# InternLM/lmdeploy

Measured on AMD Instinct MI355X. Metric: decode tokens/sec, Llama-3-8B W4A16 int8-KV batch 64 (1024-in/1k-out synthetic), higher is better.
Workload: dtype f16; 1 GPU; Llama-3-8B shapes, W4A16 AWQ g128 random weights, quant_policy=8 KV, batch 64, 1024-token random prompts, greedy decode, TP=1; batch=64, prompt_len=1024, parallelism=tp1, collectives=none, rccl_ranks=0, decode_splits=1, hipgraph=True, rmsnorm_fold=0, gemm_dispatch=measured at start-up (tm_engine_tune_gemm), prefill_rows=8192

## Files before the change

### lmdeploy_amd/csrc/c_api.hip

```cpp
#include "../../include/tm_mi355x.h"
#include "scheduler.h"
#define TM_TRY_RC(expr)          \
    do {                        \
        const int _rc = (expr); \
        if (_rc) {              \
            return _rc;         \
        }                       \
    } while (0)
#include "tm_common.h"
#include "tm_kernels.h"
#include <string.h>
#include <cmath>
#include <vector>

namespace tmk {

static thread_local std::string g_last_error;

void set_last_error(const std::string& msg)
{
    g_last_error = msg;
}
const char* get_last_error()
{
// ... 285 lines not shown

int tm_linear_dequant_f16(const tm_linear* w, void* out_nk, tm_stream_t st)
{
    TM_REQUIRE(w && out_nk, "null pointer");
    return launch_dequant_p32_f16((half_t*)out_nk, w->w, (hipStream_t)st);
}


int tm_linear_forward(const tm_linear* w, const void* x, int ldx, void* y, int ldy, int M, int gated_silu, int nt,
                      int splits, int waves, void* workspace, tm_stream_t st)
{
    TM_REQUIRE(w && x && y, "null pointer");
    GemmConfig cfg = gemm_pick_config(w->w, M);
    if (nt > 0) {
        cfg.nt = nt;
    }
    if (splits > 0) {
        cfg.splits = splits;
    }
    if (nt > 0 || (waves > 0 && !(waves & 0x200))) {
        cfg.d32_shape = -1;
        if (splits <= 0) {
            cfg.splits = gemm_pick_config_general(w->w, M).splits;
        }
    }
    if (waves > 0 && (waves & 0x200) && (waves & 0xff) == kShapeF16 && !w->w.image16) {
        TM_TRY_RC(linear_weight_build_f16_image(const_cast<tm_linear*>(w)->w, (hipStream_t)st));
    }
    if (waves > 0 && (waves & 0x200)) {
        TM_REQUIRE(dec32_supported(w->w, M), "decode kernel: u4 weights, N % 32 == 0");
        cfg.d32_shape = waves & 0xff;
        TM_REQUIRE((cfg.d32_shape >= 6 && cfg.d32_shape <= 9) || (cfg.d32_shape <= 5 && (cfg.d32_shape >= 4) == (M > 64))
                       || (cfg.d32_shape == kShapeWide2 && M <= 64)
                       || (cfg.d32_shape == kShapeLC && M <= 64) || ((cfg.d32_shape == kShapePre256 || cfg.d32_shape == kShapeF16) && M > 64)
                       || (dec32_is_merge_shape(cfg.d32_shape) && M <= 64),
                   "P32 kernel shape 0..3 / 11 (M <= 64), 4 / 5 / 12 (M > 64), 6..9 (32-row blocks, any M) or 16 + (0..3 | 6..9) "
                   "(M <= 64: split-K merged inside the launch)");
        waves = 0;
    }
    if (dec32_is_merge_shape(cfg.d32_shape) && workspace && cfg.splits > 1) {
        cfg.tickets = (unsigned*)((char*)workspace + gemm_workspace_bytes(M, w->w.N, 16));
        TM_HIP_CHECK(hipMemsetAsync(cfg.tickets, 0, 8192, (hipStream_t)st));
    }
    if (waves > 0) {
        TM_REQUIRE((waves & 0xff) == 4 || (waves & 0xff) == 8 || (waves & 0xff) == 16,
                   "waves in {4, 8, 16} (+0x100: two k-phases)");
        cfg.waves   = waves & 0xff;
        cfg.kphases = (waves & 0x100) ? 2 : 1;
    }
    TM_REQUIRE(cfg.splits <= 16, "splits <= 16");
    if (!workspace) {
        cfg.splits = 1;
    }
    return launch_linear(w->w, (const half_t*)x, ldx, (half_t*)y, ldy, M, gated_silu != 0, cfg, (float*)workspace, false,
                         nullptr, (hipStream_t)st);
}

int tm_linear_residual_norm(const tm_linear* w, const void* x, int ldx, void* y, void* resid, const void* norm_w, float eps, int M,
                            int shape, int splits, void* workspace, tm_stream_t st)
{
    TM_REQUIRE(w && x && y && resid && norm_w && workspace, "null pointer");
    const int N = w->w.N;
    GemmConfig cfg = gemm_pick_config(w->w, M);
    if (shape >= 0) {
        TM_REQUIRE(dec32_supported(w->w, M) && (shape <= 3 || (shape >= 6 && shape <= 10) || shape == kShapeLC)
                       && (M <= 64 || (M <= kFoldMaxRows && shape >= 6 && shape <= 9)),
                   "decode tile 0..3 / 6..10 / 11 at M <= 64; the 32-row-block tiles 6..9 up to 128 rows");
        cfg.d32_shape = shape;
    }
// ... 677 lines not shown
```

### lmdeploy_amd/csrc/gemm_decode.hip

```cpp
#include "tm_common.h"
#include "tm_kernels.h"
#include "p32_layout.h"
#include "gemm_decode_common.h"
#include <stdlib.h>
#include <algorithm>
#include <type_traits>
#include <map>
#include <mutex>
#include <string>
#include <tuple>
#include <stdio.h>

namespace tmk {

__global__ void repack_p32_kernel(uint32_t* __restrict__ out, const int32_t* __restrict__ qw, const half_t* __restrict__ scales,
                                  const half_t* __restrict__ zeros, int K, int N)
{
    const size_t idx   = (size_t)blockIdx.x * blockDim.x + threadIdx.x;
    const int    ncg   = N / 32;
    const size_t total = (size_t)(K / 128) * ncg * (kP32Unit / 4);
    if (idx >= total) {
        return;
    }
    const size_t unit = idx / (kP32Unit / 4);
// ... 1074 lines not shown
            }
            return launch_dec32_one<MH, 4, 4, 4, 2, kD32Mode>(p, grid, st);
        }
        case 1:
            return launch_dec32_one<MH, 8, 2, 4, 4, kD32Mode>(p, grid, st);
        case 2:
            return launch_dec32_one<MH, 4, 2, 4, 4, kD32Mode>(p, grid, st);
        case 3:
            if constexpr (l2pf_compiled) {
                if (l2pf == 1) return launch_dec32_one<MH, 2, 4, 4, 2, kD32Mode | 0x4000>(p, grid, st);
                if (l2pf == 2) return launch_dec32_one<MH, 2, 4, 4, 2, kD32Mode | 0x8000>(p, grid, st);
            }
            return launch_dec32_one<MH, 2, 4, 4, 2, kD32Mode>(p, grid, st);
        case kShapeWide2:
            return launch_dec32_one<MH, 8, 2, 2, 2, kD32Mode>(p, grid, st);
        default: break;
    }
    set_last_error("gemm_dec32: unknown shape");
    return 1;
}

static int dec32_base_shape(int shape)
{
    static const int base[4] = {3, 0, 2, 1};
    if (dec32_is_merge_shape(shape)) {
        shape -= kShapeMerge;
    }
    return shape >= 6 && shape <= 9 ? base[shape - 6] : shape;
}

static void dec32_shape_dims(int shape, int* cg, int* s)
{
    static const int cgs[6] = {4, 8, 4, 2, 8, 16};
    if (shape == kShapeLC) {
        *cg = 4;
        *s  = 4;
        return;
    }
    if (shape == kShapePre256 || shape == kShapeF16) {
        *cg = 8;
        *s  = 1;
        return;
    }
    shape = dec32_base_shape(shape);
    if (shape == kShapeWide2) {
        *cg = 8;
        *s  = 2;
        return;
    }
    *cg = cgs[shape < 0 || shape > 5 ? 0 : shape];
    *s  = shape == 5 ? 1 : (shape == 4 ? 2 : 4);
}

static bool dec32_on(bool big)
{
    static const int on     = env_int2("TM_GEMM_D32", 1);
    static const int on_big = env_int2("TM_GEMM_D32_PREFILL", 1);
    return on && (!big || on_big);
}

bool dec32_supported(const LinearWeight& w, int M)
{
    return dec32_on(M > 64) && w.type == 0 && w.packed32 != nullptr && M >= 1 && w.N % 32 == 0 && w.K % 128 == 0;
}

bool dec32_serves_every_m(int K, int N)
{
// ... 46 lines not shown
                kv.second.second, std::get<0>(kv.first));
    }
    gen_table_export_lines(f);
    fclose(f);
    return 0;
}

int dec32_table_import(const char* path)
{
    FILE* f = fopen(path, "r");
    if (!f) {
        set_last_error(std::string("cannot read ") + path);
        return 1;
    }
    int  K, N, M, shape, splits, n = 0, skipped = 0;
    char line[160];
    while (fgets(line, sizeof line, f)) {
        if (line[0] == 'G') {
            const bool ok = gen_table_import_line(line);
            n += ok ? 1 : 0;
            skipped += ok ? 0 : 1;
            continue;
        }
        if (line[0] == '#' || line[0] == '\n') {
            continue;
        }
        int       role = 0;
        const int got  = sscanf(line, "%d %d %d %d %d %d", &K, &N, &M, &shape, &splits, &role);
        if (got < 5 || role < 0 || role > 4) {
            ++skipped;
            continue;
        }
        const bool big = M > 64;
        const bool lc  = shape == kShapeLC && M <= 64;
        const bool p256 = (shape == kShapePre256 || (shape == kShapeF16 && splits == 1)) && M > 64;
        const bool mrg = dec32_is_merge_shape(shape) && M <= 64 && splits >= 2;
        const bool w2k = shape == kShapeWide2 && M <= 64;
        if (K > 0 && N > 0 && M > 0 && M == dec32_m_bucket(M) && shape >= 0 && (shape <= 9 || lc || p256 || mrg || w2k) && splits >= 1 && splits <= 16
            && (big ? shape >= 4 : (shape != 4 && shape != 5)) && !(shape == 5 && N < 512) && K % 128 == 0 && N % 32 == 0) {
            dec32_table_set(K, N, M, shape, splits, role);
            ++n;
        }
        else {
            ++skipped;
        }
    }
    fclose(f);
    if (skipped) {
        fprintf(stderr, "[tm] %s: %d dispatch line(s) not understood by this build were skipped (%d imported)\n", path, skipped, n);
    }
    return n > 0 ? 0 : 1;
}

int dec32_m_bucket(int M)
{
    if (M <= 256) {
        return M;
    }
    int b = 512;
    while (b < M && b < 8192) {
        b <<= 1;
    }
    return b;
}

int dec32_candidates(const LinearWeight& w, int M, int (*out)[2], int cap)
{
// ... 12 lines not shown
        }
        int       cgn, S;
        dec32_shape_dims(shape, &cgn, &S);
        const int tiles = (ncg + cgn - 1) / cgn * (rows32 ? (M + 31) / 32 : (shape == 4 || shape == 5) ? (M + 127) / 128 : 1);
        for (int s = 1; s <= 16; ++s) {
            int per = (KB + s - 1) / s;
            per     = (per + S - 1) / S * S;
            if ((KB + per - 1) / per != s) {
                continue;
            }
            if ((s > 1 && tiles * s > (rows32 ? 512 : 320)) || tiles * s < 32 || (M > 256 && s > 4)) {
                continue;
            }
            if (n < cap) {
                out[n][0] = shape;
                out[n][1] = s;
                ++n;
            }
        }
    }
    if (M <= 64) {
        const int base = n;
        for (int i = 0; i < base; ++i) {
            const int sh = out[i][0], sp = out[i][1];
            if (dec32_fold_shape(sh) && sh < kShapeMerge && sp >= 2 && sp <= 4 && n < cap) {
                out[n][0] = kShapeMerge + sh;
                out[n][1] = sp;
                ++n;
            }
        }
    }
    if (M <= 64) {
        const int tiles = (ncg + 3) / 4;
        for (int s = 1; s <= 16; ++s) {
            int per = (KB + s - 1) / s;
            per     = (per + 3) / 4 * 4;
            if ((KB + per - 1) / per != s || (s > 1 && tiles * s > 320) || tiles * s < 32) {
                continue;
            }
            if (n < cap) {
                out[n][0] = kShapeLC;
                out[n][1] = s;
                ++n;
            }
        }
    }
    if (M >= 1024 && M <= 8192 && w.N >= 256 && w.image16 != nullptr && n < cap) {
        out[n][0] = kShapeF16;
        out[n][1] = 1;
        ++n;
    }
    if (M >= 256 && M <= 8192 && w.N >= 256) {
        const int tiles = (ncg + 7) / 8 * ((M + 255) / 256);
        for (int s = 1; s <= 4; ++s) {
            const int per = (KB + s - 1) / s;
            if ((KB + per - 1) / per != s || (s > 1 && tiles * s > 512) || per < 8) {
                continue;
            }
            if (n < cap) {
                out[n][0] = kShapePre256;
                out[n][1] = s;
                ++n;
            }
        }
    }
    return n;
}

void dec32_pick(const LinearWeight& w, int M, int* shape_out, int* splits_out)
{
    dec32_pick_ex(w, M, shape_out, splits_out, true);
}

void dec32_pick_ex(const LinearWeight& w, int M, int* shape_out, int* splits_out, bool use_table)
{
    const int ncg = w.N / 32;
// ... 61 lines not shown
    }
    return M <= kFoldMaxRows && ((shape >= 6 && shape <= 9) || (shape == 4 && !producer));
}

bool dec32_fold_shape(int shape)
{
    if (dec32_is_merge_shape(shape)) {
        shape -= kShapeMerge;
    }
    return (shape >= 0 && shape <= 3) || (shape >= 6 && shape <= 9) || shape == kShapeWide2;
}

int launch_linear_dec32(const LinearWeight& w, const half_t* x, int ldx, half_t* y, int ldy, int M, bool gated_silu, int shape,
                        int splits, float* workspace, int* slabs_out, hipStream_t st, NormFold* nf)
{
    const bool produce = nf && nf->resid != nullptr;
    const bool consume = nf && nf->ss_in != nullptr;
    bool       merge   = false;
    if (dec32_is_merge_shape(shape)) {
        shape -= kShapeMerge;
        merge = !produce && splits > 1;
        TM_REQUIRE(!merge || (nf && nf->tickets && (M <= 64 || (M <= kFoldMaxRows && shape >= 6 && shape <= 9))),
                   "merged split-K: arrival counters (NormFold::tickets), M <= 64 (32-row-block tiles: <= 128)");
    }
    TM_REQUIRE(!nf || !(produce || consume)
                   || (M <= 64 ? dec32_fold_shape(shape) : (M <= kFoldMaxRows && ((shape >= 6 && shape <= 9) || (shape == 4 && !produce)))),
               "folded RMSNorm: decode tiles 0..3 / 6..10 at M <= 64; 32-row-block tiles 6..9 (and tile 4 as a consumer) up to 128 rows");
    TM_REQUIRE(!produce || (!gated_silu && nf->norm_w && nf->ss_out && ldy % 4 == 0), "folded RMSNorm, producer: residual, norm weight, sums");
    TM_REQUIRE(!consume || (nf->ss_tiles >= 1 && nf->inv_h > 0.f), "folded RMSNorm, consumer: tiles and 1 / H");
    TM_REQUIRE(w.packed32 != nullptr && w.N % 32 == 0, "decode GEMM: P32 layout missing");
    if (shape == kShapeF16 && (w.image16 == nullptr || M <= 64)) {
        shape = kShapePre256;
    }
    TM_REQUIRE(M >= 1 && shape >= 0 && (shape <= 9 || shape == kShapeWide2 || shape == kShapeLC || shape == kShapePre256 || shape == kShapeF16)
                   && (shape >= 6 || (M <= 64) == (shape < 4)) && (shape != kShapeLC || M <= 64) && (shape != kShapePre256 || M > 64)
                   && (shape != kShapeWide2 || M <= 64),
               "decode GEMM: shapes 0..3, 10 and 11 take M <= 64, shapes 4 / 5 / 12 take M > 64, shapes 6..9 any M");
    TM_REQUIRE(ldx % 8 == 0, "x rows must be 16-byte aligned");
    int cgn, S;
    dec32_shape_dims(shape, &cgn, &S);
    Dec32Params p{};
    p.x       = x;
    p.ldx     = ldx;
    p.wp      = shape == kShapeF16 ? (const void*)w.image16 : w.packed32;
    if (shape == kShapeF16) {
        splits = 1;
    }
    p.y       = y;
    p.ldy     = ldy;
    p.partial = workspace;
    p.M       = M;
    p.N       = w.N;
    p.K       = w.K;
    p.KB      = w.K / 128;
    p.ncg     = w.N / 32;
    int per   = (p.KB + splits - 1) / splits;
    per       = (per + S - 1) / S * S;
    per       = per > p.KB ? p.KB : per;
    splits    = (p.KB + per - 1) / per;
    TM_REQUIRE(splits == 1 || workspace != nullptr, "split-K needs a workspace");
    p.kb_per_split = per;
    merge          = merge && splits > 1;
    p.epilogue     = produce ? 3 : (splits > 1 && !merge) ? 2 : (gated_silu ? 1 : 0);
    if (merge) {
        p.merge   = 1;
        p.tickets = nf->tickets;
    }
    if (produce) {
        TM_REQUIRE(splits == 1 || nf->tickets != nullptr, "folded RMSNorm, producer with split-K: arrival counters");
        p.resid   = nf->resid;
        p.norm_w  = nf->norm_w;
        p.ss_out  = nf->ss_out;
        p.tickets = nf->tickets;
    }
    if (consume) {
        p.ss_in    = nf->ss_in;
        p.ss_tiles = nf->ss_tiles;
        p.ss_inv_h = nf->inv_h;
        p.ss_eps   = nf->eps;
    }
    static const int wt = env_int2("TM_D32_WT", 1);
    p.wt           = wt;
    dim3      grid((p.ncg + cgn - 1) / cgn, splits,
                   (shape == kShapePre256 || shape == kShapeF16) ? (M + 255) / 256 : (shape == kShapeLC || shape == kShapeWide2) ? 1 : shape >= 6 ? (M + 31) / 32 : shape >= 4 ? (M + 127) / 128 : 1);
    static const char* const role_tag[6] = {"gemm", "w_qkv", "wo", "w1w3", "w2", "lm_head"};
    p.dbg        = gemm_trace_for((size_t)grid.x * grid.y * grid.z, role_tag[w.role >= 0 && w.role <= 5 ? w.role : 0], grid.x, grid.y, grid.z);
    const int rc = shape == kShapeF16 ? launch_f16_256(p, grid, st) :
                   shape == kShapePre256 ? launch_pre256(p, grid, st) :
                   shape == kShapeLC ? launch_dec_lc(p, grid, st) :
                   shape == kShapeWide2 ? (M <= 32 ? launch_dec32_shape<1>(p, grid, shape, st) : launch_dec32_shape<2>(p, grid, shape, st)) :
                   shape >= 6 ? launch_dec32_shape<1>(p, grid, dec32_base_shape(shape), st) :
                   shape >= 4 ? launch_dec32_shape<4>(p, grid, shape, st) :
                   M <= 32    ? launch_dec32_shape<1>(p, grid, shape, st) :
                                launch_dec32_shape<2>(p, grid, shape, st);
    if (rc) {
        return rc;
    }
    if (produce) {
        nf->tiles_out = (int)grid.x;
        splits        = 1;
    }
    if (merge) {
        splits = 1;
    }
    if (slabs_out) {
        *slabs_out = splits;
    }
    return 0;
}

}
```

### lmdeploy_amd/csrc/gemm_decode_common.h

```cpp
#pragma once
#include "tm_common.h"
#include "tm_kernels.h"
#include "p32_layout.h"
#include <type_traits>

namespace tmk {

typedef float floatx16 __attribute__((ext_vector_type(16)));

struct Dec32Params {
    const half_t* x;
    int           ldx;
    const void*   wp;
    half_t*       y;
    int           ldy;
    float*        partial;
    int           M, N, K, KB, ncg;
    int           kb_per_split;
    int           epilogue;
    int           wt;
    uint64_t*     dbg;
    half_t*       resid;
    const half_t* norm_w;
    float*        ss_out;
// ... 19 lines not shown
{
    if (mode <= 1) {
        asm volatile("global_store_dwordx4 %0, %1, off sc1\n\ts_nop 1" ::"v"(dst), "v"(v) : "memory");
    }
    else if (mode == 2) {
        asm volatile("global_store_dwordx4 %0, %1, off sc0 sc1\n\ts_nop 1" ::"v"(dst), "v"(v) : "memory");
    }
    else if (mode == 3) {
        asm volatile("global_store_dwordx4 %0, %1, off nt\n\ts_nop 1" ::"v"(dst), "v"(v) : "memory");
    }
    else {
        asm volatile("global_store_dwordx4 %0, %1, off sc0 sc1 nt\n\ts_nop 1" ::"v"(dst), "v"(v) : "memory");
    }
}
__device__ __forceinline__ void store_wt(half4_t* dst, half4_t v)
{
    asm volatile("global_store_dwordx2 %0, %1, off sc1" ::"v"(dst), "v"(v) : "memory");
}
__device__ __forceinline__ void store_wt(half2_t* dst, half2_t v)
{
    asm volatile("global_store_dword %0, %1, off sc1" ::"v"(dst), "v"(v) : "memory");
}

template<int N, class F, int I = 0>
__device__ __forceinline__ void static_for(F&& f)
{
    if constexpr (I < N) {
        f(std::integral_constant<int, I>{});
        static_for<N, F, I + 1>(static_cast<F&&>(f));
    }
}

int launch_dec_lc(const Dec32Params& p, dim3 grid, hipStream_t st);
int launch_pre256(const Dec32Params& p, dim3 grid, hipStream_t st);
int launch_f16_256(const Dec32Params& p, dim3 grid, hipStream_t st);

}
```

### lmdeploy_amd/csrc/gemm_decode_lc.hip

```cpp
#include "gemm_decode_common.h"
#include <stdlib.h>

namespace tmk {

typedef float floatx2 __attribute__((ext_vector_type(2)));

__device__ __forceinline__ half8_t raw8_p32(uint32_t w)
{
    const uint32_t m = 0x000f000fu;
    return bit_cast<half8_t>(u32x4{w & m, (w >> 4) & m, (w >> 8) & m, (w >> 12) & m});
}

template<int MH, int PFS, int ABL = 0>
__global__ __launch_bounds__(768) void gemm_dec_lc_kernel(Dec32Params p)
{
    constexpr int NCW   = 2;
    constexpr int CGW   = 2;
    constexpr int WK    = 4;
    constexpr int NCONS = CGW * WK;
    constexpr int NLOAD = 4;
    constexpr int T     = (NCONS + NLOAD) * 64;
    constexpr int ROWS  = 32 * MH;
    constexpr int KBB   = ROWS * 256;
    constexpr int S     = WK;
    constexpr int STG   = S * KBB;
    constexpr int CGT   = CGW * NCW;
    constexpr int NPC   = S * ROWS / 4;
    constexpr int DR    = NPC / NLOAD;
    static_assert(NPC % NLOAD == 0, "DMA pieces per loader wave");
    static_assert(WK * ROWS * CGT * 128 <= 2 * STG, "reduction image must fit the stage buffers");

    extern __shared__ __attribute__((aligned(16))) char smem[];

    const int tid  = threadIdx.x;
    const int wgid = blockIdx.y * gridDim.x + blockIdx.x;
    if (p.dbg && tid == 0) {
        p.dbg[wgid * 8 + 0] = __builtin_amdgcn_s_memrealtime();
        p.dbg[wgid * 8 + 4] = ((uint64_t)__builtin_amdgcn_s_getreg(20 | (31 << 11)) << 32) | (uint32_t)__builtin_amdgcn_s_getreg(4 | (31 << 11));
    }
    const int lane = tid & 63;
    const int wave = __builtin_amdgcn_readfirstlane(tid >> 6);
    const int l31  = lane & 31;
    const int half = lane >> 5;

    const int kb0 = blockIdx.y * p.kb_per_split;
    const int nkb = min(p.kb_per_split, p.KB - kb0);
    const int nst = (nkb + S - 1) / S;
    const int Mloc = min(ROWS, p.M);

    const unsigned lds0 = __builtin_amdgcn_readfirstlane((unsigned)(size_t)smem);

    floatx16 acc[NCW][MH];
#pragma unroll
    for (int c = 0; c < NCW; ++c) {
// ... 193 lines not shown
                        }
                    }
                    if constexpr (!(ABL & (1 | 2))) {
#pragma unroll
                        for (int g = 0; g < 2 * MH; ++g) {
                            __builtin_amdgcn_sched_group_barrier(0x008, 1, 0);
                            __builtin_amdgcn_sched_group_barrier(0x002, MH == 2 ? 7 : 14, 0);
                        }
                    }
                    __builtin_amdgcn_sched_barrier(0);
                });
                if constexpr (!(ABL & 16)) {
                    LC_LOAD_W(u, (t + PFS) * S + wk);
                }
                __builtin_amdgcn_s_barrier();
            };
            int t0 = 0;
            for (; t0 + PFS <= nst; t0 += PFS) {
                static_for<PFS>([&](auto U) { stage(U, t0 + decltype(U)::value); });
            }
            static_for<PFS>([&](auto U) {
                if (t0 + decltype(U)::value < nst) {
                    stage(U, t0 + decltype(U)::value);
                }
            });
        }
#undef LC_LOAD_W
    }
    if (p.dbg && tid == 0) {
        p.dbg[wgid * 8 + 2] = __builtin_amdgcn_s_memrealtime();
        p.dbg[wgid * 8 + 6] = __builtin_amdgcn_s_memtime();
    }

    {
        constexpr int C4  = CGT * 8;
        floatx4*      red = (floatx4*)smem;
        if (wave < NCONS) {
#pragma unroll
            for (int c = 0; c < NCW; ++c) {
#pragma unroll
                for (int h = 0; h < MH; ++h) {
                    const int m = 32 * h + l31;
#pragma unroll
                    for (int g4 = 0; g4 < 4; ++g4) {
                        const int c4 = (cw * NCW + c) * 8 + 2 * g4 + half;
                        red[(wk * ROWS + m) * C4 + (c4 ^ (m & 7))] =
                            floatx4{acc[c][h][4 * g4], acc[c][h][4 * g4 + 1], acc[c][h][4 * g4 + 2], acc[c][h][4 * g4 + 3]};
                    }
                }
            }
        }
        __syncthreads();
        if (p.dbg && tid == 0) {
            p.dbg[wgid * 8 + 7] = __builtin_amdgcn_s_memrealtime();
        }
        constexpr int NE    = ROWS * C4;
        const int     ncol0 = blockIdx.x * CGT * 32;
#pragma unroll
        for (int e0 = 0; e0 < NE; e0 += T) {
            const int e = e0 + tid;
            if (NE % T != 0 && e >= NE) {
                break;
            }
            const int m  = e / C4;
            const int c4 = e % C4;
            floatx4   a  = red[m * C4 + (c4 ^ (m & 7))];
#pragma unroll
            for (int k = 1; k < WK; ++k) {
                a += red[(k * ROWS + m) * C4 + (c4 ^ (m & 7))];
            }
            const int n = ncol0 + c4 * 4;
            if (m >= Mloc || n >= p.N) {
                continue;
            }
            if (p.epilogue == 2) {
                floatx4* dst = (floatx4*)(p.partial + ((size_t)blockIdx.y * p.M + m) * p.N + n);
                if (p.wt & 1) {
                    store_wt(dst, a, p.wt >> 4);
                }
                else {
                    *dst = a;
                }
            }
            else if (p.epilogue == 1) {
                const float s0 = a[0] / (1.0f + __builtin_expf(-a[0]));
                const float s1 = a[2] / (1.0f + __builtin_expf(-a[2]));
                half2_t     o  = {(half_t)(s0 * a[1]), (half_t)(s1 * a[3])};
                half2_t*    dst = (half2_t*)(p.y + (size_t)m * p.ldy + (n >> 1));
                if (p.wt & 2) {
                    store_wt(dst, o);
                }
                else {
                    *dst = o;
                }
            }
            else {
                half4_t  o   = {(half_t)a[0], (half_t)a[1], (half_t)a[2], (half_t)a[3]};
                half4_t* dst = (half4_t*)(p.y + (size_t)m * p.ldy + n);
                if (p.wt & 2) {
                    store_wt(dst, o);
                }
                else {
                    *dst = o;
                }
            }
        }
    }
    if (p.dbg && tid == 0) {
        asm volatile("s_waitcnt vmcnt(0)" ::: "memory");
        p.dbg[wgid * 8 + 3] = __builtin_amdgcn_s_memrealtime();
    }
}

template<int MH, int PFS, int ABL = 0>
static int launch_lc_one(const Dec32Params& p, dim3 grid, hipStream_t st)
{
    constexpr int lds = 2 * 4 * 32 * MH * 256;
    if (const int rc = ensure_dynamic_lds((const void*)gemm_dec_lc_kernel<MH, PFS, ABL>, lds)) {
        return rc;
    }
    gemm_dec_lc_kernel<MH, PFS, ABL><<<grid, 768, lds, st>>>(p);
    TM_HIP_CHECK(hipGetLastError());
    return 0;
}

int launch_dec_lc(const Dec32Params& p, dim3 grid, hipStream_t st)
{
    static const int pfs = []() {
        const char* v = getenv("TM_LC_PFS");
        return v ? atoi(v) : 3;
    }();
#ifdef TM_EXPERIMENTS
    static const int abl = []() {
        const char* v = getenv("TM_D32_ABL");
        return v ? atoi(v) : -1;
    }();
    if (p.M > 32) {
        switch (abl) {
#define LC_CASE(v) case v: return launch_lc_one<2, 3, v>(p, grid, st)
            LC_CASE(0x20); LC_CASE(0x40); LC_CASE(0xc0); LC_CASE(0xe0); LC_CASE(1); LC_CASE(2); LC_CASE(4); LC_CASE(8); LC_CASE(16); LC_CASE(7); LC_CASE(15); LC_CASE(24); LC_CASE(31);
#undef LC_CASE
            default: break;
        }
    }
// ... 9 lines not shown
```

### lmdeploy_amd/csrc/tm_kernels.h

```cpp
#pragma once
#include <stdio.h>
#include "tm_common.h"
#include <vector>

namespace tmk {

struct KvLayout {
    int kv_heads;
    int head_dim;
    int block_len;
    int bits;
    __host__ __device__ int token_data_size() const { return bits * head_dim / 8; }
    __host__ __device__ int token_param_size() const { return bits < 16 ? 4 : 0; }
    __host__ __device__ int head_data_size() const { return block_len * token_data_size(); }
    __host__ __device__ int head_param_size() const { return block_len * token_param_size(); }
    __host__ __device__ int layer_size() const
    {
        return kv_heads * 2 * head_data_size() + kv_heads * 2 * head_param_size();
    }
    __host__ __device__ int k_data(int head, int ti) const { return head * 2 * head_data_size() + ti * token_data_size(); }
    __host__ __device__ int v_data(int head, int ti) const { return k_data(head, ti) + head_data_size(); }
    __host__ __device__ int k_param(int head, int ti) const
    {
        return kv_heads * 2 * head_data_size() + head * 2 * head_param_size() + ti * token_param_size();
// ... 61 lines not shown
    int           batch;
    int           max_q_len;
    int           q_heads;
    int           kv_heads;
    float         scale_log2;
};
int launch_prefill_attention(const PrefillAttnParams& p, hipStream_t st);

struct LinearWeight {
    int       K = 0, N = 0, group = 128;
    int       type = 0;
    int       role = 0;
    void*     packed = nullptr;
    uint32_t* sz     = nullptr;
    size_t    packed_bytes = 0, sz_bytes = 0;
    void*     packed32 = nullptr;
    size_t    packed32_bytes = 0;
    void*     packed8 = nullptr;
    size_t    packed8_bytes = 0;
    half_t*   image16 = nullptr;
};
struct GemmConfig {
    int nt;
    int splits;
    int waves;
    int kphases;
    int kstage;
    int d32_shape = -1;
    unsigned* tickets = nullptr;
};
constexpr int kShapePre256     = 12;
constexpr int kShapeF16        = 13;
constexpr int kShapeLC         = 11;
constexpr int kShapeMerge      = 16;
constexpr int kShapeWide2      = 10;
inline bool dec32_is_merge_shape(int shape)
{
    const int b = shape - kShapeMerge;
    return (b >= 0 && b <= 3) || (b >= 6 && b <= 10);
}
int    linear_weight_prepare_u4(LinearWeight& w, const int32_t* qweight , const half_t* scales,
                                const half_t* zeros, hipStream_t st, bool p32_only = false);
bool   dec32_serves_every_m(int K, int N);
int    linear_weight_prepare_f16(LinearWeight& w, const half_t* weight , hipStream_t st);
int    linear_weight_prepare_fp8(LinearWeight& w, const uint8_t* weight , const float* block_scales ,
                                 bool gated_scales , hipStream_t st);
void   linear_weight_free(LinearWeight& w);
int    linear_weight_build_f16_image(LinearWeight& w, hipStream_t st);
int    launch_dequant_p32_f16(half_t* out_nk , const LinearWeight& w, hipStream_t st);
size_t gemm_workspace_bytes(int M, int N, int splits);
size_t gemm_general_image_bytes(int K, int N, int type);
constexpr size_t kGeneralImageLimit = (size_t)1 << 31;
int    launch_splitk_reduce(half_t* y, int ldy, const float* partial, int splits, int M, int N, bool gated, hipStream_t st);
GemmConfig gemm_pick_config(const LinearWeight& w, int M);
GemmConfig gemm_pick_config_general(const LinearWeight& w, int M);
int launch_linear(const LinearWeight& w, const half_t* x, int ldx, half_t* y, int ldy, int M, bool gated_silu,
                  GemmConfig cfg, float* workspace, bool defer_reduce, int* slabs, hipStream_t st);

size_t p32_bytes(int K, int N);
int    launch_repack_p32(void* out, const int32_t* qweight, const half_t* scales, const half_t* zeros, int K, int N, hipStream_t st);
bool   dec32_supported(const LinearWeight& w, int M);
void   dec32_pick(const LinearWeight& w, int M, int* shape_out, int* splits_out);
void   dec32_pick_ex(const LinearWeight& w, int M, int* shape_out, int* splits_out, bool use_table);
void   dec32_table_set(int K, int N, int M, int shape, int splits, int role = 0);
bool   dec32_table_get(int K, int N, int M, int* shape, int* splits, int role = 0);
void   dec32_table_clear();
// ... 143 lines not shown
```

Baseline: 19220 tokens/s.

## Add LDS-DMA multi-buffered decode GEMM variant as tunable candidate shape

Adds a new decode GEMM kernel (shape 14) that streams activations and packed int4 weights straight into LDS via buffer_load...lds, using multi-stage ring buffers with dedicated loader waves and vmcnt-based pipelining. Consumer waves dequantize from LDS and run MFMA, and the reduction epilogue is factored into a shared helper. The new shape is added to the start-up autotuner's candidate list for M<=64, so it is picked only if measured faster. The cost is extra tuning time plus more complexity from hand-written inline asm and barriers.

```diff
diff --git a/lmdeploy_amd/csrc/c_api.hip b/lmdeploy_amd/csrc/c_api.hip
--- a/lmdeploy_amd/csrc/c_api.hip
+++ b/lmdeploy_amd/csrc/c_api.hip
@@ -341,9 +341,9 @@
         cfg.d32_shape = waves & 0xff;
         TM_REQUIRE((cfg.d32_shape >= 6 && cfg.d32_shape <= 9) || (cfg.d32_shape <= 5 && (cfg.d32_shape >= 4) == (M > 64))
                        || (cfg.d32_shape == kShapeWide2 && M <= 64)
-                       || (cfg.d32_shape == kShapeLC && M <= 64) || ((cfg.d32_shape == kShapePre256 || cfg.d32_shape == kShapeF16) && M > 64)
+                       || ((cfg.d32_shape == kShapeLC || cfg.d32_shape == kShapeLCW) && M <= 64) || ((cfg.d32_shape == kShapePre256 || cfg.d32_shape == kShapeF16) && M > 64)
                        || (dec32_is_merge_shape(cfg.d32_shape) && M <= 64),
-                   "P32 kernel shape 0..3 / 11 (M <= 64), 4 / 5 / 12 (M > 64), 6..9 (32-row blocks, any M) or 16 + (0..3 | 6..9) "
+                   "P32 kernel shape 0..3 / 11 / 14 (M <= 64), 4 / 5 / 12 (M > 64), 6..9 (32-row blocks, any M) or 16 + (0..3 | 6..9) "
                    "(M <= 64: split-K merged inside the launch)");
         waves = 0;
     }
diff --git a/lmdeploy_amd/csrc/gemm_decode.hip b/lmdeploy_amd/csrc/gemm_decode.hip
--- a/lmdeploy_amd/csrc/gemm_decode.hip
+++ b/lmdeploy_amd/csrc/gemm_decode.hip
@@ -1130,7 +1130,7 @@
 static void dec32_shape_dims(int shape, int* cg, int* s)
 {
     static const int cgs[6] = {4, 8, 4, 2, 8, 16};
-    if (shape == kShapeLC) {
+    if (shape == kShapeLC || shape == kShapeLCW) {
         *cg = 4;
         *s  = 4;
         return;
@@ -1243,7 +1243,7 @@
             continue;
         }
         const bool big = M > 64;
-        const bool lc  = shape == kShapeLC && M <= 64;
+        const bool lc  = (shape == kShapeLC || shape == kShapeLCW) && M <= 64;
         const bool p256 = (shape == kShapePre256 || (shape == kShapeF16 && splits == 1)) && M > 64;
         const bool mrg = dec32_is_merge_shape(shape) && M <= 64 && splits >= 2;
         const bool w2k = shape == kShapeWide2 && M <= 64;
@@ -1322,16 +1322,18 @@
     }
     if (M <= 64) {
         const int tiles = (ncg + 3) / 4;
-        for (int s = 1; s <= 16; ++s) {
-            int per = (KB + s - 1) / s;
-            per     = (per + 3) / 4 * 4;
-            if ((KB + per - 1) / per != s || (s > 1 && tiles * s > 320) || tiles * s < 32) {
-                continue;
-            }
-            if (n < cap) {
-                out[n][0] = kShapeLC;
-                out[n][1] = s;
-                ++n;
+        for (const int shape : {kShapeLC, kShapeLCW}) {
+            for (int s = 1; s <= 16; ++s) {
+                int per = (KB + s - 1) / s;
+                per     = (per + 3) / 4 * 4;
+                if ((KB + per - 1) / per != s || (s > 1 && tiles * s > 320) || tiles * s < 32) {
+                    continue;
+                }
+                if (n < cap) {
+                    out[n][0] = shape;
+                    out[n][1] = s;
+                    ++n;
+                }
             }
         }
     }
@@ -1459,10 +1461,11 @@
     if (shape == kShapeF16 && (w.image16 == nullptr || M <= 64)) {
         shape = kShapePre256;
     }
-    TM_REQUIRE(M >= 1 && shape >= 0 && (shape <= 9 || shape == kShapeWide2 || shape == kShapeLC || shape == kShapePre256 || shape == kShapeF16)
-                   && (shape >= 6 || (M <= 64) == (shape < 4)) && (shape != kShapeLC || M <= 64) && (shape != kShapePre256 || M > 64)
+    const bool lc = shape == kShapeLC || shape == kShapeLCW;
+    TM_REQUIRE(M >= 1 && shape >= 0 && (shape <= 9 || shape == kShapeWide2 || lc || shape == kShapePre256 || shape == kShapeF16)
+                   && (shape >= 6 || (M <= 64) == (shape < 4)) && (!lc || M <= 64) && (shape != kShapePre256 || M > 64)
                    && (shape != kShapeWide2 || M <= 64),
-               "decode GEMM: shapes 0..3, 10 and 11 take M <= 64, shapes 4 / 5 / 12 take M > 64, shapes 6..9 any M");
+               "decode GEMM: shapes 0..3, 10, 11 and 14 take M <= 64, shapes 4 / 5 / 12 take M > 64, shapes 6..9 any M");
     TM_REQUIRE(ldx % 8 == 0, "x rows must be 16-byte aligned");
     int cgn, S;
     dec32_shape_dims(shape, &cgn, &S);
@@ -1509,12 +1512,13 @@
     static const int wt = env_int2("TM_D32_WT", 1);
     p.wt           = wt;
     dim3      grid((p.ncg + cgn - 1) / cgn, splits,
-                   (shape == kShapePre256 || shape == kShapeF16) ? (M + 255) / 256 : (shape == kShapeLC || shape == kShapeWide2) ? 1 : shape >= 6 ? (M + 31) / 32 : shape >= 4 ? (M + 127) / 128 : 1);
+                   (shape == kShapePre256 || shape == kShapeF16) ? (M + 255) / 256 : (lc || shape == kShapeWide2) ? 1 : shape >= 6 ? (M + 31) / 32 : shape >= 4 ? (M + 127) / 128 : 1);
     static const char* const role_tag[6] = {"gemm", "w_qkv", "wo", "w1w3", "w2", "lm_head"};
     p.dbg        = gemm_trace_for((size_t)grid.x * grid.y * grid.z, role_tag[w.role >= 0 && w.role <= 5 ? w.role : 0], grid.x, grid.y, grid.z);
     const int rc = shape == kShapeF16 ? launch_f16_256(p, grid, st) :
                    shape == kShapePre256 ? launch_pre256(p, grid, st) :
                    shape == kShapeLC ? launch_dec_lc(p, grid, st) :
+                   shape == kShapeLCW ? launch_dec_lcw(p, grid, st) :
                    shape == kShapeWide2 ? (M <= 32 ? launch_dec32_shape<1>(p, grid, shape, st) : launch_dec32_shape<2>(p, grid, shape, st)) :
                    shape >= 6 ? launch_dec32_shape<1>(p, grid, dec32_base_shape(shape), st) :
                    shape >= 4 ? launch_dec32_shape<4>(p, grid, shape, st) :
diff --git a/lmdeploy_amd/csrc/gemm_decode_common.h b/lmdeploy_amd/csrc/gemm_decode_common.h
--- a/lmdeploy_amd/csrc/gemm_decode_common.h
+++ b/lmdeploy_amd/csrc/gemm_decode_common.h
@@ -75,6 +75,7 @@
 }
 
 int launch_dec_lc(const Dec32Params& p, dim3 grid, hipStream_t st);
+int launch_dec_lcw(const Dec32Params& p, dim3 grid, hipStream_t st);
 int launch_pre256(const Dec32Params& p, dim3 grid, hipStream_t st);
 int launch_f16_256(const Dec32Params& p, dim3 grid, hipStream_t st);
 
diff --git a/lmdeploy_amd/csrc/gemm_decode_lc.hip b/lmdeploy_amd/csrc/gemm_decode_lc.hip
--- a/lmdeploy_amd/csrc/gemm_decode_lc.hip
+++ b/lmdeploy_amd/csrc/gemm_decode_lc.hip
@@ -9,6 +9,87 @@
 {
     const uint32_t m = 0x000f000fu;
     return bit_cast<half8_t>(u32x4{w & m, (w >> 4) & m, (w >> 8) & m, (w >> 12) & m});
+}
+
+template<int MH>
+__device__ __forceinline__ void lc_reduce_store(const Dec32Params& p, char* smem, const floatx16 (&acc)[2][MH], const bool consumer, const int cw,
+                                                const int wk, const int wgid)
+{
+    constexpr int NCW = 2, CGW = 2, WK = 4, CGT = CGW * NCW, T = 768, ROWS = 32 * MH;
+    const int tid = threadIdx.x, lane = tid & 63, l31 = lane & 31, half = lane >> 5;
+    const int Mloc = min(ROWS, p.M);
+    constexpr int C4  = CGT * 8;
+    floatx4*      red = (floatx4*)smem;
+    if (consumer) {
+#pragma unroll
+        for (int c = 0; c < NCW; ++c) {
+#pragma unroll
+            for (int h = 0; h < MH; ++h) {
+                const int m = 32 * h + l31;
+#pragma unroll
+                for (int g4 = 0; g4 < 4; ++g4) {
+                    const int c4 = (cw * NCW + c) * 8 + 2 * g4 + half;
+                    red[(wk * ROWS + m) * C4 + (c4 ^ (m & 7))] =
+                        floatx4{acc[c][h][4 * g4], acc[c][h][4 * g4 + 1], acc[c][h][4 * g4 + 2], acc[c][h][4 * g4 + 3]};
+                }
+            }
+        }
+    }
+    __syncthreads();
+    if (p.dbg && tid == 0) {
+        p.dbg[wgid * 8 + 7] = __builtin_amdgcn_s_memrealtime();
+    }
+    constexpr int NE    = ROWS * C4;
+    const int     ncol0 = blockIdx.x * CGT * 32;
+#pragma unroll
+    for (int e0 = 0; e0 < NE; e0 += T) {
+        const int e = e0 + tid;
+        if (NE % T != 0 && e >= NE) {
+            break;
+        }
+        const int m  = e / C4;
+        const int c4 = e % C4;
+        floatx4   a  = red[m * C4 + (c4 ^ (m & 7))];
+#pragma unroll
+        for (int k = 1; k < WK; ++k) {
+            a += red[(k * ROWS + m) * C4 + (c4 ^ (m & 7))];
+        }
+        const int n = ncol0 + c4 * 4;
+        if (m >= Mloc || n >= p.N) {
+            continue;
+        }
+        if (p.epilogue == 2) {
+            floatx4* dst = (floatx4*)(p.partial + ((size_t)blockIdx.y * p.M + m) * p.N + n);
+            if (p.wt & 1) {
+                store_wt(dst, a, p.wt >> 4);
+            }
+            else {
+                *dst = a;
+            }
+        }
+        else if (p.epilogue == 1) {
+            const float s0 = a[0] / (1.0f + __builtin_expf(-a[0]));
+            const float s1 = a[2] / (1.0f + __builtin_expf(-a[2]));
+            half2_t     o  = {(half_t)(s0 * a[1]), (half_t)(s1 * a[3])};
+            half2_t*    dst = (half2_t*)(p.y + (size_t)m * p.ldy + (n >> 1));
+            if (p.wt & 2) {
+                store_wt(dst, o);
+            }
+            else {
+                *dst = o;
+            }
+        }
+        else {
+            half4_t  o   = {(half_t)a[0], (half_t)a[1], (half_t)a[2], (half_t)a[3]};
+            half4_t* dst = (half4_t*)(p.y + (size_t)m * p.ldy + n);
+            if (p.wt & 2) {
+                store_wt(dst, o);
+            }
+            else {
+                *dst = o;
+            }
+        }
+    }
 }
 
 template<int MH, int PFS, int ABL = 0>
@@ -19,7 +100,6 @@
     constexpr int WK    = 4;
     constexpr int NCONS = CGW * WK;
     constexpr int NLOAD = 4;
-    constexpr int T     = (NCONS + NLOAD) * 64;
     constexpr int ROWS  = 32 * MH;
     constexpr int KBB   = ROWS * 256;
     constexpr int S     = WK;
@@ -279,84 +359,270 @@
         p.dbg[wgid * 8 + 6] = __builtin_amdgcn_s_memtime();
     }
 
-    {
-        constexpr int C4  = CGT * 8;
-        floatx4*      red = (floatx4*)smem;
-        if (wave < NCONS) {
-#pragma unroll
-            for (int c = 0; c < NCW; ++c) {
-#pragma unroll
-                for (int h = 0; h < MH; ++h) {
-                    const int m = 32 * h + l31;
-#pragma unroll
-                    for (int g4 = 0; g4 < 4; ++g4) {
-                        const int c4 = (cw * NCW + c) * 8 + 2 * g4 + half;
-                        red[(wk * ROWS + m) * C4 + (c4 ^ (m & 7))] =
-                            floatx4{acc[c][h][4 * g4], acc[c][h][4 * g4 + 1], acc[c][h][4 * g4 + 2], acc[c][h][4 * g4 + 3]};
-                    }
-                }
-            }
-        }
-        __syncthreads();
-        if (p.dbg && tid == 0) {
-            p.dbg[wgid * 8 + 7] = __builtin_amdgcn_s_memrealtime();
-        }
-        constexpr int NE    = ROWS * C4;
-        const int     ncol0 = blockIdx.x * CGT * 32;
-#pragma unroll
-        for (int e0 = 0; e0 < NE; e0 += T) {
-            const int e = e0 + tid;
-            if (NE % T != 0 && e >= NE) {
-                break;
-            }
-            const int m  = e / C4;
-            const int c4 = e % C4;
-            floatx4   a  = red[m * C4 + (c4 ^ (m & 7))];
-#pragma unroll
-            for (int k = 1; k < WK; ++k) {
-                a += red[(k * ROWS + m) * C4 + (c4 ^ (m & 7))];
-            }
-            const int n = ncol0 + c4 * 4;
-            if (m >= Mloc || n >= p.N) {
-                continue;
-            }
-            if (p.epilogue == 2) {
-                floatx4* dst = (floatx4*)(p.partial + ((size_t)blockIdx.y * p.M + m) * p.N + n);
-                if (p.wt & 1) {
-                    store_wt(dst, a, p.wt >> 4);
-                }
-                else {
-                    *dst = a;
-                }
-            }
-            else if (p.epilogue == 1) {
-                const float s0 = a[0] / (1.0f + __builtin_expf(-a[0]));
-                const float s1 = a[2] / (1.0f + __builtin_expf(-a[2]));
-                half2_t     o  = {(half_t)(s0 * a[1]), (half_t)(s1 * a[3])};
-                half2_t*    dst = (half2_t*)(p.y + (size_t)m * p.ldy + (n >> 1));
-                if (p.wt & 2) {
-                    store_wt(dst, o);
-                }
-                else {
-                    *dst = o;
-                }
-            }
-            else {
-                half4_t  o   = {(half_t)a[0], (half_t)a[1], (half_t)a[2], (half_t)a[3]};
-                half4_t* dst = (half4_t*)(p.y + (size_t)m * p.ldy + n);
-                if (p.wt & 2) {
-                    store_wt(dst, o);
-                }
-                else {
-                    *dst = o;
-                }
-            }
-        }
-    }
+    lc_reduce_store<MH>(p, smem, acc, wave < NCONS, cw, wk, wgid);
     if (p.dbg && tid == 0) {
         asm volatile("s_waitcnt vmcnt(0)" ::: "memory");
         p.dbg[wgid * 8 + 3] = __builtin_amdgcn_s_memrealtime();
     }
+}
+
+template<bool NT, class R>
+__device__ __forceinline__ void lds_dma16(const int voff, const R rs, const unsigned dst, const int soff)
+{
+    unsigned keep;
+    if constexpr (NT) {
+        asm volatile("s_mov_b32 %0, m0\n\ts_mov_b32 m0, %3\n\ts_nop 0\n\t"
+                     "buffer_load_dwordx4 %1, %2, %4 offen nt lds\n\ts_mov_b32 m0, %0"
+                     : "=&s"(keep)
+                     : "v"(voff), "s"(rs), "s"(dst), "s"(soff)
+                     : "memory");
+    }
+    else {
+        asm volatile("s_mov_b32 %0, m0\n\ts_mov_b32 m0, %3\n\ts_nop 0\n\t"
+                     "buffer_load_dwordx4 %1, %2, %4 offen lds\n\ts_mov_b32 m0, %0"
+                     : "=&s"(keep)
+                     : "v"(voff), "s"(rs), "s"(dst), "s"(soff)
+                     : "memory");
+    }
+}
+
+template<int NB, int D, class F>
+__device__ __forceinline__ void lcw_stream(const int nh, F&& issue)
+{
+    static_assert(NB >= 2 && D * (NB - 2) <= 63, "vmcnt is a 6-bit count");
+#pragma unroll
+    for (int g = 0; g < NB - 1; ++g) {
+        if (g < nh) {
+            issue(g, g);
+        }
+    }
+    if (nh >= NB - 1) {
+        asm volatile("s_waitcnt vmcnt(%0)" ::"i"(D * (NB - 2)) : "memory");
+    }
+    else {
+        asm volatile("s_waitcnt vmcnt(0)" ::: "memory");
+    }
+    __builtin_amdgcn_s_barrier();
+    int buf = NB - 1;
+    for (int h = 0; h < nh; ++h) {
+        if (h + NB - 1 < nh) {
+            issue(h + NB - 1, buf);
+            buf = buf + 1 == NB ? 0 : buf + 1;
+            asm volatile("s_waitcnt vmcnt(%0)" ::"i"(D * (NB - 2)) : "memory");
+        }
+        else {
+            asm volatile("s_waitcnt vmcnt(0)" ::: "memory");
+        }
+        __builtin_amdgcn_s_barrier();
+    }
+}
+
+template<int MH, int NBX, int NBW>
+__global__ __launch_bounds__(768) void gemm_dec_lcw_kernel(Dec32Params p)
+{
+    constexpr int NCW   = 2;
+    constexpr int CGW   = 2;
+    constexpr int WK    = 4;
+    constexpr int NCONS = CGW * WK;
+    constexpr int CGT   = CGW * NCW;
+    constexpr int ROWS  = 32 * MH;
+    constexpr int XKB   = ROWS * 128;
+    constexpr int XSB   = WK * XKB;
+    constexpr int WCB   = WK * CGT * 1024;
+    constexpr int WSB   = WCB + WK * CGT * 128;
+    constexpr int WOFF  = NBX * XSB;
+    constexpr int DX    = XSB / 1024 / 2;
+    constexpr int DW    = WK * CGT / 2 + 1;
+    static_assert(WOFF + NBW * WSB <= 160 * 1024, "LDS of a CU");
+    static_assert(WK * ROWS * CGT * 128 <= WOFF + NBW * WSB, "reduction image must fit the rings");
+
+    extern __shared__ __attribute__((aligned(16))) char smem[];
+
+    const int tid  = threadIdx.x;
+    const int wgid = blockIdx.y * gridDim.x + blockIdx.x;
+    if (p.dbg && tid == 0) {
+        p.dbg[wgid * 8 + 0] = __builtin_amdgcn_s_memrealtime();
+        p.dbg[wgid * 8 + 4] = ((uint64_t)__builtin_amdgcn_s_getreg(20 | (31 << 11)) << 32) | (uint32_t)__builtin_amdgcn_s_getreg(4 | (31 << 11));
+    }
+    const int lane = tid & 63;
+    const int wave = __builtin_amdgcn_readfirstlane(tid >> 6);
+    const int l31  = lane & 31;
+    const int half = lane >> 5;
+
+    const int kb0  = blockIdx.y * p.kb_per_split;
+    const int nkb  = min(p.kb_per_split, p.KB - kb0);
+    const int nh   = 2 * ((nkb + WK - 1) / WK);
+    const int Mloc = min(ROWS, p.M);
+
+    const unsigned lds0 = __builtin_amdgcn_readfirstlane((unsigned)(size_t)smem);
+
+    floatx16 acc[NCW][MH];
+#pragma unroll
+    for (int c = 0; c < NCW; ++c) {
+#pragma unroll
+        for (int h = 0; h < MH; ++h) {
+#pragma unroll
+            for (int r = 0; r < 16; ++r) {
+                acc[c][h][r] = 0.f;
+            }
+        }
+    }
+    const int cw = wave & (CGW - 1);
+    const int wk = wave / CGW;
+
+    if (nh > 0) {
+        if (wave >= NCONS + 2) {
+            const int  lw   = wave - NCONS - 2;
+            const auto rs_w = __builtin_amdgcn_make_buffer_rsrc((void*)p.wp, 0, (int)((size_t)p.KB * p.ncg * kP32Unit), 0x00020000);
+            const int  su   = lw * 8 + (lane >> 3);
+            const int  scg  = min((int)blockIdx.x * CGT + (su & 3), p.ncg - 1);
+            lcw_stream<NBW, DW>(nh, [&](const int g, const int buf) __attribute__((always_inline)) {
+                const int      t   = g >> 1;
+                const unsigned dst = lds0 + WOFF + buf * WSB;
+#pragma unroll
+                for (int r = 0; r < WK * CGT / 2; ++r) {
+                    const int u  = 2 * r + lw;
+                    const int so = ((kb0 + min(t * WK + (u >> 2), nkb - 1)) * p.ncg + min((int)blockIdx.x * CGT + (u & 3), p.ncg - 1)) * kP32Unit
+                                   + (g & 1) * 1024;
+                    lds_dma16<true>(lane * 16, rs_w, dst + u * 1024, so);
+                }
+                const int vo = ((kb0 + min(t * WK + (su >> 2), nkb - 1)) * p.ncg + scg) * kP32Unit + 2048 + (lane & 7) * 16;
+                lds_dma16<false>(vo, rs_w, dst + WCB + lw * 1024, 0);
+            });
+        }
+        else if (wave >= NCONS) {
+            const int  lw   = wave - NCONS;
+            const auto rs_x = __builtin_amdgcn_make_buffer_rsrc((void*)p.x, 0, (int)(((size_t)(Mloc - 1) * p.ldx + p.K) * 2), 0x00020000);
+            int        doff[DX];
+#pragma unroll
+            for (int r = 0; r < DX; ++r) {
+                const int pc  = 2 * r + lw;
+                const int kbi = pc / (ROWS / 8);
+                const int row = (pc % (ROWS / 8)) * 8 + (lane >> 3);
+                const int ch  = (lane & 7) ^ ((row >> 1) & 7);
+                doff[r]       = (min(row, Mloc - 1) * p.ldx + ch * 8) * 2 + kbi * 256;
+            }
+            lcw_stream<NBX, DX>(nh, [&](const int g, const int buf) __attribute__((always_inline)) {
+                const int so = (kb0 + (g >> 1) * WK) * 256 + (g & 1) * 128;
+#pragma unroll
+                for (int r = 0; r < DX; ++r) {
+                    lds_dma16<false>(doff[r], rs_x, lds0 + buf * XSB + (2 * r + lw) * 1024, so);
+                }
+            });
+        }
+        else {
+            const unsigned xrd = lds0 + wk * XKB + l31 * 128;
+            const int      fsw = (half ^ ((l31 >> 1) & 7)) << 4;
+            const unsigned wrd = lds0 + WOFF + (wk * CGT + cw * NCW) * 1024 + lane * 16;
+            const unsigned srd = lds0 + WOFF + WCB + (wk * CGT + cw * NCW) * 128 + l31 * 4;
+            uint32_t       m1024 = 0x64006400u, m64 = 0x54005400u;
+            asm volatile("" : "+v"(m1024), "+v"(m64));
+            __builtin_amdgcn_s_barrier();
+            if (p.dbg && tid == 0) {
+                p.dbg[wgid * 8 + 1] = __builtin_amdgcn_s_memrealtime();
+                p.dbg[wgid * 8 + 5] = __builtin_amdgcn_s_memtime();
+            }
+            int xb = 0, wb = 0;
+            for (int h = 0; h < nh; ++h) {
+                const bool     live = (h >> 1) * WK + wk < nkb;
+                const unsigned xa   = xrd + xb * XSB;
+                const unsigned wa   = wrd + wb * WSB;
+                const unsigned sa   = srd + wb * WSB;
+                u32x4          wq[NCW];
+                uint32_t       sq[NCW];
+                half8_t        f0[MH], f1[MH];
+                asm volatile("ds_read_b128 %0, %1" : "=v"(wq[0]) : "v"(wa));
+                asm volatile("ds_read_b32 %0, %1" : "=v"(sq[0]) : "v"(sa));
+                asm volatile("ds_read_b128 %0, %1 offset:1024" : "=v"(wq[1]) : "v"(wa));
+                asm volatile("ds_read_b32 %0, %1 offset:128" : "=v"(sq[1]) : "v"(sa));
+                auto rd = [&](half8_t(&f)[MH], int j) __attribute__((always_inline)) {
+                    const unsigned ad = xa + (unsigned)((32 * j) ^ fsw);
+#pragma unroll
+                    for (int hh = 0; hh < MH; ++hh) {
+                        asm volatile("ds_read_b128 %0, %1 offset:%2" : "=v"(f[hh]) : "v"(ad), "i"(hh * 32 * 128));
+                    }
+                };
+                auto wt = [&](half8_t(&f)[MH], auto N) __attribute__((always_inline)) {
+                    constexpr int n = decltype(N)::value;
+                    if constexpr (MH == 1) {
+                        asm volatile("s_waitcnt lgkmcnt(%1)" : "+v"(f[0]) : "i"(n));
+                    }
+                    else {
+                        asm volatile("s_waitcnt lgkmcnt(%2)" : "+v"(f[0]), "+v"(f[1]) : "i"(n));
+                    }
+                    __builtin_amdgcn_sched_barrier(0);
+                };
+                rd(f0, 0);
+                rd(f1, 1);
+                asm volatile("s_waitcnt lgkmcnt(%4)" : "+v"(wq[0]), "+v"(wq[1]), "+v"(sq[0]), "+v"(sq[1]) : "i"(MH));
+                half2_t s2[NCW], z2[NCW];
+#pragma unroll
+                for (int c = 0; c < NCW; ++c) {
+                    const half2_t pr = bit_cast<half2_t>(live ? sq[c] : 0u);
+                    s2[c]            = half2_t{pr[0], pr[0]};
+                    z2[c]            = half2_t{pr[1], pr[1]};
+                }
+                half8_t a0 = dequant8_p32(wq[0][0], s2[0], z2[0], m1024, m64), a1;
+                static_for<4>([&](auto J) {
+                    constexpr int  j  = decltype(J)::value;
+                    half8_t(&cur)[MH] = (j & 1) ? f1 : f0;
+                    half8_t(&nxt)[MH] = (j & 1) ? f0 : f1;
+                    if constexpr (j >= 1 && j + 1 < 4) {
+                        rd(nxt, j + 1);
+                    }
+                    wt(cur, std::integral_constant<int, (j + 1 < 4) ? MH : 0>{});
+                    a1 = dequant8_p32(wq[1][j], s2[1], z2[1], m1024, m64);
+#pragma unroll
+                    for (int hh = 0; hh < MH; ++hh) {
+                        acc[0][hh] = __builtin_amdgcn_mfma_f32_32x32x16_f16(a0, cur[hh], acc[0][hh], 0, 0, 0);
+                    }
+                    if constexpr (j + 1 < 4) {
+                        a0 = dequant8_p32(wq[0][j + 1], s2[0], z2[0], m1024, m64);
+                    }
+#pragma unroll
+                    for (int hh = 0; hh < MH; ++hh) {
+                        acc[1][hh] = __builtin_amdgcn_mfma_f32_32x32x16_f16(a1, cur[hh], acc[1][hh], 0, 0, 0);
+                    }
+#pragma unroll
+                    for (int g = 0; g < 2 * MH; ++g) {
+                        __builtin_amdgcn_sched_group_barrier(0x008, 1, 0);
+                        __builtin_amdgcn_sched_group_barrier(0x002, MH == 2 ? 7 : 14, 0);
+                    }
+                    __builtin_amdgcn_sched_barrier(0);
+                });
+                xb = xb + 1 == NBX ? 0 : xb + 1;
+                wb = wb + 1 == NBW ? 0 : wb + 1;
+                asm volatile("s_waitcnt lgkmcnt(0)" ::: "memory");
+                __builtin_amdgcn_s_barrier();
+            }
+        }
+    }
+    if (p.dbg && tid == 0) {
+        p.dbg[wgid * 8 + 2] = __builtin_amdgcn_s_memrealtime();
+        p.dbg[wgid * 8 + 6] = __builtin_amdgcn_s_memtime();
+    }
+    lc_reduce_store<MH>(p, smem, acc, wave < NCONS, cw, wk, wgid);
+    if (p.dbg && tid == 0) {
+        asm volatile("s_waitcnt vmcnt(0)" ::: "memory");
+        p.dbg[wgid * 8 + 3] = __builtin_amdgcn_s_memrealtime();
+    }
+}
+
+template<int MH, int NBX, int NBW>
+static int launch_lcw_one(const Dec32Params& p, dim3 grid, hipStream_t st)
+{
+    constexpr int lds = NBX * 4 * 32 * MH * 128 + NBW * (16 * 1024 + 16 * 128);
+    if (const int rc = ensure_dynamic_lds((const void*)gemm_dec_lcw_kernel<MH, NBX, NBW>, lds)) {
+        return rc;
+    }
+    gemm_dec_lcw_kernel<MH, NBX, NBW><<<grid, 768, lds, st>>>(p);
+    TM_HIP_CHECK(hipGetLastError());
+    return 0;
+}
+
+int launch_dec_lcw(const Dec32Params& p, dim3 grid, hipStream_t st)
+{
+    return p.M <= 32 ? launch_lcw_one<1, 3, 6>(p, grid, st) : launch_lcw_one<2, 2, 5>(p, grid, st);
 }
 
 template<int MH, int PFS, int ABL = 0>
diff --git a/lmdeploy_amd/csrc/tm_kernels.h b/lmdeploy_amd/csrc/tm_kernels.h
--- a/lmdeploy_amd/csrc/tm_kernels.h
+++ b/lmdeploy_amd/csrc/tm_kernels.h
@@ -117,6 +117,7 @@
 constexpr int kShapePre256     = 12;
 constexpr int kShapeF16        = 13;
 constexpr int kShapeLC         = 11;
+constexpr int kShapeLCW        = 14;
 constexpr int kShapeMerge      = 16;
 constexpr int kShapeWide2      = 10;
 inline bool dec32_is_merge_shape(int shape)
```

Result: no change. 19220 tokens/s, median of 3 (+0.0%).
